# ZHKKKe/PixelSSL

Hardware: NVIDIA H100
Metric: images/sec DeepLab-v2-R101 MT 513x513 bs16 (higher is better)
Workload: dtype f16x3 (fp16 pairs, fp32 accumulate)

## Files before the change

include/pixelssl_b200.h:

```cpp
#ifndef PIXELSSL_B200_H
#define PIXELSSL_B200_H

#include <stdint.h>

#ifdef __cplusplus
extern "C" {
#endif

#define PXL_ERR_BAD_ARG   (-1)
#define PXL_ERR_UNSUPPORTED (-2)

int pxl_abi_version(void);
int64_t pxl_launch_count(void);
void pxl_reset_launch_count(void);

int64_t pxl_mse_workspace_bytes(void);
int pxl_mse_consistency(const float* s, const float* t, int64_t n, float loss_scale,
                        float* loss_out, float* grad_s, void* workspace, void* stream);
int pxl_mse_consistency_bwd(const float* s, const float* t, int64_t n, float loss_scale,
                            const float* upstream, float* grad_s, void* stream);

int pxl_ce2d(const float* logits, const float* labels, int n, int C, int64_t HW, int ignore_index,
             float* per_sample, float* grad_logits, const float* upstream, float upstream_const,
             void* stream);
// ... 60 lines not shown
int pxl_bn_bwd_params(const double* dsums, int C, float* dgamma, float* dbeta, int accumulate,
                      void* stream);

int pxl_maxpool3x3s2_fwd(const float* x, float* y, int N, int H, int W, int C, int OH, int OW,
                         void* stream);
int pxl_maxpool3x3s2_bwd(const float* x, const float* y, const float* dy, float* dx,
                         int N, int H, int W, int C, int OH, int OW, void* stream);

typedef struct {
    int N, H, W, Cin;
    int OH, OW, Cout;
    int ldo;
    int mul, div;
    int ntaps;
    int precision;
} pxl_conv_geom;
#define PXL_MAX_TAPS 64
int pxl_conv_nhwc(const pxl_conv_geom* geom_host, const int* taps_dydx_host ,
                  const float* in, const float* w, const float* bias ,
                  float* out, void* stream);
int pxl_conv_wgrad_nhwc(const pxl_conv_geom* geom_host, const int* taps_dydx_host,
                        const float* in, const float* dy, float* dw, void* stream);
int pxl_conv_tc_launch(const pxl_conv_geom* geom_host, const int* taps_dydx_host, const float* in_hi,
                       const float* in_lo, const float* w_hi, const float* w_lo, const float* bias,
                       float* out, void* stream);
typedef struct {
    int w_ntaps;
    const int* widx_host;
    int out_mul, out_offy, out_offx, out_H, out_W;
    double* bn_stats;
    float out_scale;
    const float* out_scale_dev;
    int out_accumulate;
} pxl_conv_tc_ext;
int pxl_conv_tc_launch_ex(const pxl_conv_geom* geom_host, const int* taps_dydx_host, const pxl_conv_tc_ext* ext_host,
                          const float* in_hi, const float* in_lo, const float* w_hi, const float* w_lo,
                          const float* bias, float* out, void* stream);
int pxl_conv_wgrad_tc_launch(const pxl_conv_geom* geom_host, const int* taps_dydx_host, const float* in_hi,
                             const float* in_lo, const float* dy_hi, const float* dy_lo, float* dw,
                             void* stream);
int pxl_conv_h16_launch(const pxl_conv_geom* geom_host, const int* taps_dydx_host, const pxl_conv_tc_ext* ext_host,
                        const void* in_hi, const void* in_lo, const void* w_hi, const void* w_lo,
                        const float* bias, float* out, void* stream);
int pxl_conv_wgrad_h16_launch(const pxl_conv_geom* geom_host, const int* taps_dydx_host, const void* in_hi,
                              const void* in_lo, const void* dy_hi, const void* dy_lo, float* dw, float out_scale,
                              const float* out_scale_dev, void* stream);
int pxl_h16_split(const float* x, void* hi, void* lo, int64_t n, float scale, float* slot, int target_log2,
                  void* stream);
int pxl_h16_absmax(const float* x, int64_t n, float* slot, void* stream);
int* pxl_h16_sat_counter(void);
int pxl_h16_status(void);
int pxl_h16_status_sites(int* out4_host);
int pxl_h16_reset_status(void);
int pxl_split_tf32(const float* x, float* hi, float* lo, int64_t n, void* stream);
int pxl_conv_tc_status(void);
int pxl_conv_transpose_weights(const float* w, float* wt, int Cout, int T, int Cin, void* stream);
int pxl_conv_transpose_weights_batched(const float* src_base, float* dst_base, const int64_t* table, int n,
                                       int64_t total_tiles, void* stream);
int pxl_bias_grad(const float* dy, int64_t rows, int Cout, int ldo, float* dbias, int accumulate,
                  void* stream);

int pxl_stem_conv7x7s2(const float* img_planar, const float* w, float* out, int N, int H, int W,
                       int OH, int OW, void* stream);
int pxl_stem_conv7x7s2_wgrad(const float* img_planar, const float* dy, float* dw, int N, int H, int W,
                             int OH, int OW, void* stream);
int pxl_stem_im2col(const float* img_planar, float* cols, int N, int H, int W, int OH, int OW, void* stream);

// ... 88 lines not shown
```

pixelssl_b200/_lib.py:

```python
import ctypes
import os

_HERE = os.path.dirname(os.path.abspath(__file__))
LIB_PATH = os.path.join(_HERE, 'lib', 'libpixelssl_b200.so')

c_void_p, c_int, c_int64, c_float, c_double = (ctypes.c_void_p, ctypes.c_int, ctypes.c_int64,
                                               ctypes.c_float, ctypes.c_double)


class ConvGeom(ctypes.Structure):
    _fields_ = [('N', c_int), ('H', c_int), ('W', c_int), ('Cin', c_int),
                ('OH', c_int), ('OW', c_int), ('Cout', c_int), ('ldo', c_int),
                ('mul', c_int), ('div', c_int), ('ntaps', c_int), ('precision', c_int)]


class ConvTcExt(ctypes.Structure):
    _fields_ = [('w_ntaps', c_int), ('widx_host', ctypes.POINTER(c_int)), ('out_mul', c_int),
                ('out_offy', c_int), ('out_offx', c_int), ('out_H', c_int), ('out_W', c_int),
                ('bn_stats', c_void_p), ('out_scale', c_float), ('out_scale_dev', c_void_p), ('out_accumulate', c_int)]


P = c_void_p
SIGNATURES = {
    'pxl_abi_version': (c_int, []),
    'pxl_launch_count': (c_int64, []),
    'pxl_reset_launch_count': (None, []),
    'pxl_mse_workspace_bytes': (c_int64, []),
    'pxl_mse_consistency': (c_int, [P, P, c_int64, c_float, P, P, P, P]),
    'pxl_mse_consistency_bwd': (c_int, [P, P, c_int64, c_float, P, P, P]),
    'pxl_ce2d': (c_int, [P, P, c_int, c_int, c_int64, c_int, P, P, P, c_float, P]),
    'pxl_cps_ce': (c_int, [P, P, P, P, c_int, c_int, c_int64, c_float, P, P, P, P]),
    'pxl_unimatch_ce': (c_int, [P, P, P, P, P, c_int, c_int, c_int, c_int, c_int, c_int, c_float, c_float, c_float, c_float,
                                P, P, P, P]),
    'pxl_softmax_planar': (c_int, [P, P, c_int, c_int, c_int64, P]),
    'pxl_softmax_planar_bwd': (c_int, [P, P, P, c_int, c_int, c_int64, P]),
    'pxl_softmax_mse': (c_int, [P, P, c_int, c_int, c_int64, c_float, P, P, P, P, P]),
    'pxl_bilinear_fwd': (c_int, [P, P, c_int, c_int, c_int, c_int, c_int, c_int, c_int, c_int, c_int, P]),
    'pxl_bilinear_bwd': (c_int, [P, P, c_int, c_int, c_int, c_int, c_int, c_int, c_int, c_int, c_int, P]),
    'pxl_cutmix_mix': (c_int, [P, P, P, P, c_int, c_int, c_int64, P]),
    'pxl_cutmix_confidence': (c_int, [P, c_int, c_int, c_int64, c_float, P, P]),
    'pxl_bn_stats': (c_int, [P, c_int64, c_int, P, P]),
    'pxl_bn_finalize': (c_int, [P, c_double, c_int, P, P, P, P, c_float, c_float, c_int, P, P, P, P, P]),
    'pxl_bn_eval_coeffs': (c_int, [c_int, P, P, P, P, c_float, P, P, P]),
    'pxl_bn_apply': (c_int, [P, P, P, P, c_int, P, c_int64, c_int, P]),
    'pxl_bn_bwd_reduce': (c_int, [P, P, P, P, P, c_int, c_int64, c_int, P, P, P, P]),
    'pxl_bn_bwd_dx': (c_int, [P, P, P, P, P, P, P, c_double, c_int, P, P, c_int64, c_int, P, P, P, P, P]),
    'pxl_bn_finalize_apply': (c_int, [P, P, c_double, P, P, P, P, c_float, c_float, c_int, P, P, P, P, P, c_int, P, c_int64,
                                      c_int, P]),
    'pxl_bn_bwd_params': (c_int, [P, c_int, P, P, c_int, P]),
    'pxl_bn_apply_h16': (c_int, [P, P, P, P, c_int, P, c_int64, c_int, P, P, c_float, P, P]),
    'pxl_bn_finalize_apply_h16': (c_int, [P, P, c_double, P, P, P, P, c_float, c_float, c_int, P, P, P, P, P, c_int, P, c_int64,
                                          c_int, P, P, c_float, P, P]),
    'pxl_bn_bwd_reduce_h16': (c_int, [P, P, P, P, P, c_int, c_int64, c_int, P, P, P, P, P, P]),
    'pxl_bn_bwd_dx_h16': (c_int, [P, P, P, P, P, P, P, c_double, c_int, P, P, c_int64, c_int, P, P, P, P, P, P, P, c_int, P, P]),
    'pxl_maxpool3x3s2_fwd': (c_int, [P, P, c_int, c_int, c_int, c_int, c_int, c_int, P]),
    'pxl_maxpool3x3s2_bwd': (c_int, [P, P, P, P, c_int, c_int, c_int, c_int, c_int, c_int, P]),
    'pxl_conv_nhwc': (c_int, [ctypes.POINTER(ConvGeom), ctypes.POINTER(c_int), P, P, P, P, P]),
    'pxl_conv_wgrad_nhwc': (c_int, [ctypes.POINTER(ConvGeom), ctypes.POINTER(c_int), P, P, P, P]),
    'pxl_conv_tc_launch': (c_int, [ctypes.POINTER(ConvGeom), ctypes.POINTER(c_int), P, P, P, P, P, P, P]),
    'pxl_conv_tc_launch_ex': (c_int, [ctypes.POINTER(ConvGeom), ctypes.POINTER(c_int), ctypes.POINTER(ConvTcExt), P, P, P, P, P, P, P]),
    'pxl_conv_wgrad_tc_launch': (c_int, [ctypes.POINTER(ConvGeom), ctypes.POINTER(c_int), P, P, P, P, P, P]),
    'pxl_conv_h16_launch': (c_int, [ctypes.POINTER(ConvGeom), ctypes.POINTER(c_int), ctypes.POINTER(ConvTcExt), P, P, P, P, P, P, P]),
    'pxl_conv_wgrad_h16_launch': (c_int, [ctypes.POINTER(ConvGeom), ctypes.POINTER(c_int), P, P, P, P, P, c_float, P, P]),
    'pxl_h16_split': (c_int, [P, P, P, c_int64, c_float, P, c_int, P]),
    'pxl_h16_absmax': (c_int, [P, c_int64, P, P]),
    'pxl_h16_sat_counter': (c_void_p, []),
    'pxl_h16_status': (c_int, []),
    'pxl_h16_status_sites': (c_int, [P]),
    'pxl_h16_reset_status': (c_int, []),
    'pxl_split_tf32': (c_int, [P, P, P, c_int64, P]),
    'pxl_conv_tc_status': (c_int, []),
    'pxl_conv_transpose_weights': (c_int, [P, P, c_int, c_int, c_int, P]),
    'pxl_conv_transpose_weights_batched': (c_int, [P, P, P, c_int, c_int64, P]),
    'pxl_bias_grad': (c_int, [P, c_int64, c_int, c_int, P, c_int, P]),
    'pxl_stem_conv7x7s2': (c_int, [P, P, P, c_int, c_int, c_int, c_int, c_int, P]),
    'pxl_stem_conv7x7s2_wgrad': (c_int, [P, P, P, c_int, c_int, c_int, c_int, c_int, P]),
    'pxl_stem_im2col': (c_int, [P, P, c_int, c_int, c_int, c_int, c_int, P]),
    'pxl_planar_to_nhwc': (c_int, [P, P, c_int, c_int, c_int64, c_int, c_int, P]),
    'pxl_nhwc_to_planar': (c_int, [P, P, c_int, c_int, c_int64, c_int, c_int, P]),
    'pxl_onehot_nhwc': (c_int, [P, P, c_int64, c_int, c_int, c_int, P]),
    'pxl_leaky_relu_fwd': (c_int, [P, P, c_int64, c_float, P]),
    'pxl_leaky_relu_bwd': (c_int, [P, P, P, c_int64, c_float, P]),
    'pxl_bce_logits_masked': (c_int, [P, P, c_float, c_int, c_int, c_int64, P, P, P, c_float, P]),
    'pxl_adam': (c_int, [P, P, P, P, c_int64, c_float, c_float, c_float, c_float, c_float, c_int, P]),
    'pxl_gauss_blur_sep': (c_int, [P, P, P, c_int, c_int, c_int, c_int, P, c_float, P]),
    'pxl_dilate3x3_reflect': (c_int, [P, P, c_int, c_int, c_int, P]),
    'pxl_minmax_norm': (c_int, [P, P, c_int, c_int64, c_float, c_float, c_float, P]),
    'pxl_gct_dcgt': (c_int, [P, P, P, P, c_float, c_int, c_int, c_int64, P, P, P, P]),
    'pxl_fdgt_absdiff': (c_int, [P, P, c_float, c_int, c_int, c_int64, P, P]),
    'pxl_pixel_shuffle2_nhwc': (c_int, [P, P, c_int, c_int, c_int, c_int, c_int, c_int, c_int, P]),
    'pxl_perturb_nhwc': (c_int, [P, P, P, P, P, c_int, c_int64, c_int, P]),
    'pxl_fp_dup_nhwc': (c_int, [P, P, P, c_int, c_int64, c_int, P]),
    'pxl_fp_dup_bwd_nhwc': (c_int, [P, P, P, c_int, c_int64, c_int, P]),
    'pxl_channel_mean_nhwc': (c_int, [P, P, c_int64, c_int, P]),
# ... 74 lines not shown
```

pixelssl_b200/csrc/common.cuh:

```cuda
#pragma once
#include <cuda_runtime.h>
#include <stdint.h>
#include "../../include/pixelssl_b200.h"

#define PXL_NUM_SMS 132

extern "C" void pxl_count_launch_(int n);

#define PXL_WS_WGRAD 0
#define PXL_WS_BIAS 1
#define PXL_WS_CE 2
#define PXL_WS_CPS 3
#define PXL_WS_UNIMATCH 4
#define PXL_WS_STRONG_AUG 5
#define PXL_WS_PURPOSES 6
#define PXL_WS_STREAMS 8
extern "C" void* pxl_workspace_(int purpose, void* stream, size_t bytes, int* rc);

#define PXL_CHECK_LAUNCH()                                   \
    do {                                                     \
        pxl_count_launch_(1);                                \
        cudaError_t e__ = cudaPeekAtLastError();             \
        if (e__ != cudaSuccess) return (int)e__;             \
    } while (0)

static inline int64_t pxl_cdiv(int64_t a, int64_t b) { return (a + b - 1) / b; }

#define PXL_PDL_SYNC()                                                   \
    do {                                                                 \
        asm volatile("griddepcontrol.launch_dependents;" ::: "memory");  \
        asm volatile("griddepcontrol.wait;" ::: "memory");               \
    } while (0)

extern "C" int pxl_pdl_enabled_(void);

template <typename... KArgs, typename... Args>
static inline cudaError_t pxl_launch_pdl(void (*kernel)(KArgs...), dim3 grid, dim3 block, size_t smem, cudaStream_t st,
                                         Args&&... args) {
    cudaLaunchConfig_t cfg = {};
    cfg.gridDim = grid; cfg.blockDim = block; cfg.dynamicSmemBytes = smem; cfg.stream = st;
    cudaLaunchAttribute at[1];
    at[0].id = cudaLaunchAttributeProgrammaticStreamSerialization;
    at[0].val.programmaticStreamSerializationAllowed = 1;
    cfg.attrs = at; cfg.numAttrs = pxl_pdl_enabled_() ? 1 : 0;
    return cudaLaunchKernelEx(&cfg, kernel, static_cast<KArgs>(args)...);
}

__device__ __forceinline__ float warp_sum(float v) {
// ... 36 lines not shown
```

pixelssl_b200/csrc/conv_tc.cu:

```cuda
#include "common.cuh"
#include <cuda.h>
#include <cstdlib>
#include <type_traits>

typedef CUresult (*EncodeTiledFn)(CUtensorMap*, CUtensorMapDataType, cuuint32_t, void*, const cuuint64_t*,
                                  const cuuint64_t*, const cuuint32_t*, const cuuint32_t*, CUtensorMapInterleave,
                                  CUtensorMapSwizzle, CUtensorMapL2promotion, CUtensorMapFloatOOBfill);
static EncodeTiledFn get_encode() {
    static EncodeTiledFn fn = nullptr;
    if (!fn) {
        void* p = nullptr;
        cudaDriverEntryPointQueryResult q;
        if (cudaGetDriverEntryPoint("cuTensorMapEncodeTiled", &p, cudaEnableDefault, &q) == cudaSuccess &&
            q == cudaDriverEntryPointSuccess)
            fn = (EncodeTiledFn)p;
    }
    return fn;
}

static int make_act_map(CUtensorMap* m, const void* base, int C, int W, int H, int N, int bw, int bh, int estride = 1, int f16 = 0) {
    EncodeTiledFn enc = get_encode();
    if (!enc) return PXL_ERR_UNSUPPORTED;
    const cuuint64_t eb = f16 ? 2 : 4;
    cuuint64_t dims[4] = {(cuuint64_t)C, (cuuint64_t)W, (cuuint64_t)H, (cuuint64_t)N};
// ... 158 lines not shown
#pragma unroll
    for (int k = 0; k < 4; ++k) wgmma_op<BN, F16>(part, da + 2 * k, db + 2 * k, k);
    if (split3) {
#pragma unroll
        for (int k = 0; k < 4; ++k) wgmma_op<BN, F16>(corr, dal + 2 * k, db + 2 * k, k);
#pragma unroll
        for (int k = 0; k < 4; ++k) wgmma_op<BN, F16>(corr, da + 2 * k, dbl + 2 * k, 1);
    }
}

__device__ __forceinline__ float4 tf32_split4(float4 v, float4& lo) {
    float4 h;
    const float* vp = &v.x; float* hp = &h.x; float* lp = &lo.x;
#pragma unroll
    for (int e = 0; e < 4; ++e) {
        uint32_t u;
        asm("cvt.rna.tf32.f32 %0, %1;" : "=r"(u) : "f"(vp[e]));
        u &= 0xFFFFE000u;
        hp[e] = __uint_as_float(u);
        lp[e] = vp[e] - hp[e];
    }
    return h;
}

struct TcParams {
    int Cin, Cout, ldo, ntaps, kchunks;
    int N, OH, OW;
    int BW, BH, tilesW, tilesH;
    int stages, nsplit;
    int a_inkernel;
    int in_mul;
    int out_mul, out_offy, out_offx, outH, outW;
    int ntilesN, pix_tiles, total_tiles;
    int kc;
    float out_scale;
    int out_acc;
    short dy[PXL_MAX_TAPS], dx[PXL_MAX_TAPS], widx[PXL_MAX_TAPS];
};

#define TC_A_BYTES (128 * 128)
#define TC_MAX_STAGES 8
#define TC_THREADS 384

__device__ __forceinline__ void tc_tile_coords(const TcParams& p, int tile, int bn, int& n0, int& w0, int& h0, int& n) {
    const int nt = tile / p.pix_tiles, pix = tile - nt * p.pix_tiles;
    const int tw = pix % p.tilesW, th = (pix / p.tilesW) % p.tilesH;
    n = pix / (p.tilesW * p.tilesH);
    w0 = tw * p.BW; h0 = th * p.BH; n0 = nt * bn;
}

template <int BN, int F16>
__global__ void __launch_bounds__(TC_THREADS, 1)
conv_wg_kernel(const __grid_constant__ CUtensorMap mapA, const __grid_constant__ CUtensorMap mapAlo,
               const __grid_constant__ CUtensorMap mapB, const __grid_constant__ CUtensorMap mapBlo,
               const TcParams p, const float* __restrict__ bias, float* __restrict__ out,
               double* __restrict__ stats, int* __restrict__ err_flag, const float* __restrict__ oscale_ptr) {
    extern __shared__ __align__(1024) uint8_t smem_raw[];
    __shared__ uint64_t full_bar[TC_MAX_STAGES], empty_bar[TC_MAX_STAGES];
    __shared__ float st_warp[2][8][BN];

    uint8_t* smem = (uint8_t*)(((uintptr_t)smem_raw + 1023) & ~(uintptr_t)1023);
    constexpr int B_BYTES = BN * 128;
    constexpr int PER_OP = TC_A_BYTES + B_BYTES;
    const int stage_bytes = PER_OP * (p.nsplit == 3 ? 2 : 1);
    const int iters = p.ntaps * p.kchunks;

    if (threadIdx.x == 0) {
        for (int s = 0; s < p.stages; ++s) { mbar_init(&full_bar[s], 1); mbar_init(&empty_bar[s], 256); }
        asm volatile("fence.mbarrier_init.release.cluster;" ::: "memory");
    }
    __syncthreads();
    PXL_PDL_SYNC();

    if (threadIdx.x < 128) {
        asm volatile("setmaxnreg.dec.sync.aligned.u32 40;" ::: "memory");
        if (threadIdx.x >= 32) return;
        uint32_t tx = (uint32_t)((p.BW * p.BH * 128 + B_BYTES) * (p.nsplit == 3 ? 2 : 1));
        if (p.a_inkernel) tx -= (uint32_t)(p.BW * p.BH * 128);
        uint32_t s = 0, ph = 0;
        bool ok = true;
        for (int tile = blockIdx.x; tile < p.total_tiles && ok; tile += gridDim.x) {
            int n0, w0, h0, n;
            tc_tile_coords(p, tile, BN, n0, w0, h0, n);
            int tap = 0, c0 = 0;
            for (int it = 0; it < iters; ++it) {
                ok = __all_sync(0xffffffffu, mbar_wait(&empty_bar[s], ph ^ 1u, err_flag, 1));
                if (!ok) break;
                uint8_t* sa = smem + (size_t)s * stage_bytes;
                const int ax = w0 * p.in_mul + p.dx[tap], ay = h0 * p.in_mul + p.dy[tap];
// ... 73 lines not shown
            } else {
                asm volatile("wgmma.wait_group.sync.aligned 1;" ::: "memory");
                fence_regs(corr);
                if (it > 0) {
                    mbar_arrive(&empty_bar[prev]);
#pragma unroll
                    for (int i = 0; i < BN / 2; ++i) acc[i] += corr[i];
                }
                wg_arrive();
                fence_regs(corr);
#pragma unroll
                for (int k = 2; k < 4; ++k) wgmma_op<BN, 1>(corr, da + 2 * k, db + 2 * k, k - 2);
                wg_commit();
                asm volatile("wgmma.wait_group.sync.aligned 1;" ::: "memory");
                fence_regs(part);
#pragma unroll
                for (int i = 0; i < BN / 2; ++i) acc[i] += part[i];
            }
            prev = s;
            if (++s == (uint32_t)p.stages) { s = 0; ph ^= 1u; }
        }
        if (!S3) {
            wg_wait0();
            fence_regs(corr);
            mbar_arrive(&empty_bar[prev]);
#pragma unroll
            for (int i = 0; i < BN / 2; ++i) acc[i] += corr[i];
        }
        return true;
    };
    for (int tile = blockIdx.x; tile < p.total_tiles && ok; tile += gridDim.x) {
        int n0, w0, h0, n;
        tc_tile_coords(p, tile, BN, n0, w0, h0, n);
        if (stats && n0 != st_n0) { flush_stats(); st_n0 = n0; }
#pragma unroll
        for (int i = 0; i < BN / 2; ++i) acc[i] = 0.f;
        if constexpr (F16 != 0) ok = split3 ? f16_tile(std::true_type{}) : f16_tile(std::false_type{});
        else for (int it = 0; it < iters; ++it) {
            ok = __all_sync(0xffffffffu, mbar_wait(&full_bar[s], ph, err_flag, 2));
            if (!ok) break;
            uint8_t* sa = smem + (size_t)s * stage_bytes;
            if (p.a_inkernel) {
                float4* a_hi = reinterpret_cast<float4*>(sa + cw * (TC_A_BYTES / 2));
                float4* a_lo = reinterpret_cast<float4*>(sa + PER_OP + cw * (TC_A_BYTES / 2));
#pragma unroll
                for (int c = 0; c < TC_A_BYTES / 2 / 16 / 128; ++c) {
                    float4 lo;
                    const float4 hi = tf32_split4(a_hi[t + c * 128], lo);
                    a_hi[t + c * 128] = hi;
                    a_lo[t + c * 128] = lo;
                }
                fence_async_smem();
                named_bar(2 + cw, 128);
            }
            const uint32_t sa32 = smem_base + s * (uint32_t)stage_bytes;
            const uint32_t arow = (uint32_t)cw * (TC_A_BYTES / 2);
            const uint64_t da = sw128_desc(sa32 + arow), db = sw128_desc(sa32 + TC_A_BYTES);
            const uint64_t dal = sw128_desc(sa32 + PER_OP + arow), dbl = sw128_desc(sa32 + PER_OP + TC_A_BYTES);
            wg_arrive();
            fence_regs(part);
            fence_regs(corr);
#pragma unroll
            for (int k = 0; k < 2; ++k) wgmma_op<BN, F16>(part, da + 2 * k, db + 2 * k, k);
            if (split3) {
#pragma unroll
                for (int k = 0; k < 4; ++k) wgmma_op<BN, F16>(corr, dal + 2 * k, db + 2 * k, k);
#pragma unroll
// ... 53 lines not shown
                } else if (c1ok && vec2) {
                    *reinterpret_cast<float2*>(o) = make_float2(v[h][0], v[h][1]);
                } else {
                    if (c0ok) o[0] = v[h][0];
                    if (c1ok) o[1] = v[h][1];
                }
            }
            if (stats) {
                float s0 = (valid[0] ? v[0][0] : 0.f) + (valid[1] ? v[1][0] : 0.f);
                float s1 = (valid[0] ? v[0][1] : 0.f) + (valid[1] ? v[1][1] : 0.f);
                float q0 = (valid[0] ? v[0][0] * v[0][0] : 0.f) + (valid[1] ? v[1][0] * v[1][0] : 0.f);
                float q1 = (valid[0] ? v[0][1] * v[0][1] : 0.f) + (valid[1] ? v[1][1] * v[1][1] : 0.f);
#pragma unroll
                for (int o = 4; o < 32; o <<= 1) {
                    s0 += __shfl_xor_sync(0xffffffffu, s0, o); s1 += __shfl_xor_sync(0xffffffffu, s1, o);
                    q0 += __shfl_xor_sync(0xffffffffu, q0, o); q1 += __shfl_xor_sync(0xffffffffu, q1, o);
                }
                if (lane < 4) {
                    const int slot = cw * 4 + warp;
                    st_warp[0][slot][cl] = s0; st_warp[0][slot][cl + 1] = s1;
                    st_warp[1][slot][cl] = q0; st_warp[1][slot][cl + 1] = q1;
                }
            }
        }
        if (stats) {
            named_bar(1, 256);
            if (ct < BN) {
#pragma unroll
                for (int w8 = 0; w8 < 8; ++w8) { st_s += st_warp[0][w8][ct]; st_q += st_warp[1][w8][ct]; }
            }
            named_bar(1, 256);
        }
    }
    if (stats && ok) flush_stats();
}

__global__ void __launch_bounds__(256)
split_tf32_kernel(const float4* __restrict__ x, float4* __restrict__ hi, float4* __restrict__ lo, int64_t n4) {
    const int64_t stride = (int64_t)gridDim.x * blockDim.x;
    for (int64_t i = (int64_t)blockIdx.x * blockDim.x + threadIdx.x; i < n4; i += stride) {
        float4 l;
        hi[i] = tf32_split4(__ldcs(x + i), l);
        lo[i] = l;
    }
}

extern "C" int pxl_split_tf32(const float* x, float* hi, float* lo, int64_t n, void* stream) {
    if (!x || !hi || !lo || n <= 0 || (n & 3)) return PXL_ERR_BAD_ARG;
    const int64_t n4 = n / 4;
    int blocks = (int)(pxl_cdiv(n4, 256 * 2) < PXL_NUM_SMS * 8 ? pxl_cdiv(n4, 256 * 2) : PXL_NUM_SMS * 8);
    split_tf32_kernel<<<blocks, 256, 0, (cudaStream_t)stream>>>((const float4*)x, (float4*)hi, (float4*)lo, n4);
    PXL_CHECK_LAUNCH();
    return 0;
}

static int* g_err_flag = nullptr;

static int ensure_err_flag() {
    if (g_err_flag) return 0;
    cudaError_t e = cudaMalloc(&g_err_flag, sizeof(int));
    if (e != cudaSuccess) return (int)e;
    e = cudaMemset(g_err_flag, 0, sizeof(int));
    return e == cudaSuccess ? 0 : (int)e;
}

template <typename K>
static int query_dyn_smem_limit(K kernel) {
    int dev = 0, optin = 0;
    cudaFuncAttributes a;
    if (cudaGetDevice(&dev) != cudaSuccess || cudaDeviceGetAttribute(&optin, cudaDevAttrMaxSharedMemoryPerBlockOptin, dev) != cudaSuccess ||
        cudaFuncGetAttributes(&a, kernel) != cudaSuccess)
        return 0;
    return optin - (int)a.sharedSizeBytes;
}

static void pick_tile(int OH, int OW, bool flat, int& BW, int& BH) {
    if (flat) { BW = 128; BH = 1; return; }
    double best = -1.0;
    BW = 16; BH = 8;
    for (int bw = 4; bw <= 128 && bw <= 256; ++bw) {
        int bh = 128 / bw;
        if (bh < 1) break;
        if (bh > 256) bh = 256;
        const int64_t tiles = (int64_t)((OW + bw - 1) / bw) * ((OH + bh - 1) / bh);
        const double eff = (double)OH * OW / ((double)tiles * 128.0);
        if (eff > best + 1e-9) { best = eff; BW = bw; BH = bh; }
    }
}

template <int BN, int F16>
static int fwd_smem_limit() {
    static const int v = query_dyn_smem_limit(conv_wg_kernel<BN, F16>);
    return v;
}

template <int BN, int F16>
static int launch_fwd(const CUtensorMap& mA, const CUtensorMap& mAlo, const CUtensorMap& mB, const CUtensorMap& mBlo,
                      const TcParams& p, size_t smem, cudaStream_t st, const float* bias, float* out, double* stats,
                      const float* oscale_ptr) {
    static bool attr = false;
    if (!attr) {
        cudaError_t e = cudaFuncSetAttribute(conv_wg_kernel<BN, F16>, cudaFuncAttributeMaxDynamicSharedMemorySize, fwd_smem_limit<BN, F16>());
        if (e != cudaSuccess) return (int)e;
        attr = true;
    }
    const unsigned nblk = (unsigned)(p.total_tiles < PXL_NUM_SMS ? p.total_tiles : PXL_NUM_SMS);
    cudaError_t le = pxl_launch_pdl(conv_wg_kernel<BN, F16>, dim3(nblk), dim3(TC_THREADS), smem, st, mA, mAlo, mB, mBlo, p,
                                    bias, out, stats, g_err_flag, oscale_ptr);
    if (le != cudaSuccess) return (int)le;
    PXL_CHECK_LAUNCH();
    return 0;
}

static int conv_tc_launch_core(const pxl_conv_geom* g, const int* taps, const pxl_conv_tc_ext* ext,
                               const void* in_hi, const void* in_lo, const void* w_hi, const void* w_lo,
                               const float* bias, float* out, void* stream);

extern "C" int pxl_conv_tc_launch(const pxl_conv_geom* g, const int* taps, const float* in_hi, const float* in_lo,
                                  const float* w_hi, const float* w_lo, const float* bias, float* out, void* stream) {
    if (g && g->precision > 2) return PXL_ERR_BAD_ARG;
    return conv_tc_launch_core(g, taps, nullptr, in_hi, in_lo, w_hi, w_lo, bias, out, stream);
}

extern "C" int pxl_conv_tc_launch_ex(const pxl_conv_geom* g, const int* taps, const pxl_conv_tc_ext* ext,
                                     const float* in_hi, const float* in_lo, const float* w_hi, const float* w_lo,
                                     const float* bias, float* out, void* stream) {
    if (g && g->precision > 2) return PXL_ERR_BAD_ARG;
    return conv_tc_launch_core(g, taps, ext, in_hi, in_lo, w_hi, w_lo, bias, out, stream);
}

extern "C" int pxl_conv_h16_launch(const pxl_conv_geom* g, const int* taps, const pxl_conv_tc_ext* ext,
                                   const void* in_hi, const void* in_lo, const void* w_hi, const void* w_lo,
                                   const float* bias, float* out, void* stream) {
    if (!g || (g->precision != 3 && g->precision != 4)) return PXL_ERR_BAD_ARG;
    return conv_tc_launch_core(g, taps, ext, in_hi, in_lo, w_hi, w_lo, bias, out, stream);
}

static int conv_tc_launch_core(const pxl_conv_geom* g, const int* taps, const pxl_conv_tc_ext* ext,
                               const void* in_hi, const void* in_lo, const void* w_hi, const void* w_lo,
                               const float* bias, float* out, void* stream) {
    if (!g || !taps || !in_hi || !w_hi || !out) return PXL_ERR_BAD_ARG;
    if ((g->mul != 1 && g->mul != 2) || g->div != 1) return PXL_ERR_UNSUPPORTED;
    const int f16 = g->precision >= 3 ? 1 : 0;
    const int kc = f16 ? 64 : 32;
    if (g->Cin % kc != 0 || g->ntaps > PXL_MAX_TAPS) return PXL_ERR_UNSUPPORTED;
    const int wtaps = ext && ext->w_ntaps > 0 ? ext->w_ntaps : g->ntaps;
    const int nsplit = (g->precision == 2 || g->precision == 3) ? 3 : 1;
    if (nsplit == 3 && !w_lo) return PXL_ERR_BAD_ARG;
    if (f16 && nsplit == 3 && !in_lo) return PXL_ERR_BAD_ARG;
    const int a_inkernel = (!f16 && nsplit == 3 && !in_lo) ? 1 : 0;
    const int omul = (ext && ext->out_mul > 0) ? ext->out_mul : 1;
    const bool has_out_xform = ext && (omul != 1 || ext->out_offy != 0 || ext->out_offx != 0);
    bool flat = (g->ntaps == 1 && taps[0] == 0 && taps[1] == 0 && g->OH == g->H && g->OW == g->W && g->mul == 1 &&
                 !has_out_xform);
    TcParams p;
    p.Cin = g->Cin; p.Cout = g->Cout; p.ldo = g->ldo; p.ntaps = g->ntaps; p.kchunks = g->Cin / kc;
    p.nsplit = nsplit; p.a_inkernel = a_inkernel; p.kc = kc;
    p.out_scale = (ext && ext->out_scale != 0.f) ? ext->out_scale : 1.f;
    const float* oscale_ptr = ext ? ext->out_scale_dev : nullptr;
    for (int t = 0; t < g->ntaps; ++t) {
        p.dy[t] = (short)taps[2 * t]; p.dx[t] = (short)taps[2 * t + 1];
        p.widx[t] = (short)((ext && ext->widx_host) ? ext->widx_host[t] : t);
        if (p.widx[t] < 0 || p.widx[t] >= wtaps) return PXL_ERR_BAD_ARG;
    }
    p.in_mul = g->mul;
    p.out_mul = omul; p.out_offy = has_out_xform ? ext->out_offy : 0; p.out_offx = has_out_xform ? ext->out_offx : 0;
    int mapW, mapH, mapN;
    if (flat) {
        const int64_t M = (int64_t)g->N * g->H * g->W;
        if (M >= (1ll << 31)) return PXL_ERR_UNSUPPORTED;
        p.N = 1; p.OH = 1; p.OW = (int)M;
        mapW = (int)M; mapH = 1; mapN = 1;
        p.outH = 1; p.outW = (int)M;
    } else {
        p.N = g->N; p.OH = g->OH; p.OW = g->OW;
        mapW = g->W; mapH = g->H; mapN = g->N;
        p.outH = has_out_xform ? ext->out_H : g->OH; p.outW = has_out_xform ? ext->out_W : g->OW;
    }
    pick_tile(p.OH, p.OW, flat, p.BW, p.BH);
    if (g->mul == 2 && (p.BW > 128 || p.BH > 128)) return PXL_ERR_UNSUPPORTED;
    const int BN = g->Cout > 64 ? 128 : (g->Cout > 32 ? 64 : 32);
    const int stage_bytes = (TC_A_BYTES + BN * 128) * (nsplit == 3 ? 2 : 1);
    p.tilesW = (p.OW + p.BW - 1) / p.BW; p.tilesH = (p.OH + p.BH - 1) / p.BH;
    p.pix_tiles = p.N * p.tilesH * p.tilesW;
    p.ntilesN = (g->Cout + BN - 1) / BN;
    const int64_t n_tiles = (int64_t)p.pix_tiles * p.ntilesN;
    if (n_tiles >= (1ll << 31)) return PXL_ERR_UNSUPPORTED;
    p.total_tiles = (int)n_tiles;
    const int smem_limit = f16 ? (BN == 128 ? fwd_smem_limit<128, 1>() : BN == 64 ? fwd_smem_limit<64, 1>() : fwd_smem_limit<32, 1>())
                               : (BN == 128 ? fwd_smem_limit<128, 0>() : BN == 64 ? fwd_smem_limit<64, 0>() : fwd_smem_limit<32, 0>());
    if (smem_limit <= 0) return PXL_ERR_UNSUPPORTED;
    p.stages = (smem_limit - 1024) / stage_bytes;
    if (p.stages > TC_MAX_STAGES) p.stages = TC_MAX_STAGES;
    if (p.stages < 2) return PXL_ERR_UNSUPPORTED;
    const size_t smem = (size_t)p.stages * stage_bytes + 1024;

    CUtensorMap mA, mAlo, mB, mBlo;
    int rc = make_act_map(&mA, in_hi, g->Cin, mapW, mapH, mapN, p.BW, p.BH, g->mul, f16);
    if (rc) return rc;
    rc = make_w_map(&mB, w_hi, (int64_t)wtaps * g->Cin, g->Cout, BN, f16);
    if (rc) return rc;
    if (nsplit == 3) {
        if (a_inkernel) mAlo = mA;
        else {
            rc = make_act_map(&mAlo, in_lo, g->Cin, mapW, mapH, mapN, p.BW, p.BH, g->mul, f16);
            if (rc) return rc;
        }
        rc = make_w_map(&mBlo, w_lo, (int64_t)wtaps * g->Cin, g->Cout, BN, f16);
        if (rc) return rc;
    } else {
        mAlo = mA; mBlo = mB;
    }
    p.out_acc = (ext && ext->out_accumulate) ? 1 : 0;
    if ((rc = ensure_err_flag())) return rc;
    cudaStream_t st = (cudaStream_t)stream;
    double* st_ptr = ext ? (double*)ext->bn_stats : nullptr;
    if (f16) {
        if (BN == 128) return launch_fwd<128, 1>(mA, mAlo, mB, mBlo, p, smem, st, bias, out, st_ptr, oscale_ptr);
        if (BN == 64) return launch_fwd<64, 1>(mA, mAlo, mB, mBlo, p, smem, st, bias, out, st_ptr, oscale_ptr);
        return launch_fwd<32, 1>(mA, mAlo, mB, mBlo, p, smem, st, bias, out, st_ptr, oscale_ptr);
    }
    if (BN == 128) return launch_fwd<128, 0>(mA, mAlo, mB, mBlo, p, smem, st, bias, out, st_ptr, oscale_ptr);
    if (BN == 64) return launch_fwd<64, 0>(mA, mAlo, mB, mBlo, p, smem, st, bias, out, st_ptr, oscale_ptr);
    return launch_fwd<32, 0>(mA, mAlo, mB, mBlo, p, smem, st, bias, out, st_ptr, oscale_ptr);
}

extern "C" int pxl_conv_tc_status(void) {
    if (!g_err_flag) return 0;
    int v = 0;
    if (cudaMemcpy(&v, g_err_flag, sizeof(int), cudaMemcpyDeviceToHost) != cudaSuccess) return -1;
    return v;
}

extern "C" int pxl_conv_tc_impl(const pxl_conv_geom* g, const int* taps, const float* in, const float* w,
                                const float* bias, float* out, void* stream) {
    if (!g) return PXL_ERR_BAD_ARG;
    if (g->precision == 2) return PXL_ERR_UNSUPPORTED;
    return pxl_conv_tc_launch(g, taps, in, nullptr, w, nullptr, bias, out, stream);
}

struct WgParams {
    int Cin, Cout, ldo, ntaps;
    int N, OH, OW, mul;
    int BW, BH, tilesW, tilesH, rows, rows_alloc;
    int stages, nsplit;
    int inkernel;
    int slab_ch;
    float out_scale;
    int tiles_ci, ktiles_per_cta, ktiles_total;
    short dy[PXL_MAX_TAPS], dx[PXL_MAX_TAPS];
};

template <int BN, int F16>
__global__ void __launch_bounds__(TC_THREADS, 1)
conv_wgrad_wg_kernel(const __grid_constant__ CUtensorMap mapDy, const __grid_constant__ CUtensorMap mapDyLo,
                     const __grid_constant__ CUtensorMap mapX, const __grid_constant__ CUtensorMap mapXLo,
                     const WgParams p, float* __restrict__ dw, float* __restrict__ ws, int* __restrict__ err_flag,
// ... 386 lines not shown
```

pixelssl_b200/ops.py:

```python
import ctypes
import functools

import torch

from . import _lib
from ._lib import ConvGeom, ConvTcExt, call
from .nn.peer import MAX_VALUES as _PEER_MAX_VALUES

CL = torch.channels_last
PRECISION = {'fp32': 0, 'tf32': 1, 'tf32x3': 2, 'f16x3': 3, 'f16': 4}
H16_FALLBACK = {3: 2, 4: 1}
H16_ACT_SCALE = 16.0
H16_W_SCALE = 256.0
H16_GRAD_TARGET_LOG2 = 14
_conv_precision = 0


def set_conv_precision(name):
    global _conv_precision
    _conv_precision = PRECISION[name]


def get_conv_precision():
    return _conv_precision
# ... 561 lines not shown
    return transpose_weights(w, *shape) if transposed else w


@functools.lru_cache(maxsize=None)
def conv_route(direction, Cin, Cout, mul, div, precision):
    if direction == 'wgrad':
        strides_ok, chans = div == 1 and mul in (1, 2), (Cin, Cout)
    else:
        strides_ok, chans = (div == 1 and mul in (1, 2)) or (div == 2 and mul == 1), (Cin,)
    if precision >= 3:
        if strides_ok and all(c % 64 == 0 for c in chans):
            return 'h16', precision
        precision = H16_FALLBACK[precision]
    if precision != 0 and strides_ok and all(c % 32 == 0 for c in chans):
        return 'tc', precision
    return 'ffma', 0


def _stride2_dgrad_classes(taps, ntaps):
    classes = []
    for py in (0, 1):
        for px in (0, 1):
            sub, widx = [], []
            for t in range(ntaps):
                dy, dx = taps[2 * t], taps[2 * t + 1]
                if (py + dy) % 2 == 0 and (px + dx) % 2 == 0:
                    sub += [(py + dy) // 2, (px + dx) // 2]
                    widx.append(t)
            classes.append((py, px, sub, widx))
    return classes


def conv_raw(x, w_packed, bias, taps, N, H, W, Cin, OH, OW, Cout, ldo, mul, div, out=None, precision=None, bn_stats=None,
             accumulate=False):
    ntaps = len(taps) // 2
    family, prec = conv_route('fwd', Cin, Cout, mul, div, _conv_precision if precision is None else precision)
    if family != 'h16' and (isinstance(x, H16) or isinstance(w_packed, H16)):
        raise ValueError('fp16-pair operands given for a shape the f16 wgmma kernel does not cover')
    if out is None:
        out = torch.empty((N, ldo, OH, OW), dtype=torch.float32, device=(x[0] if isinstance(x, tuple) else x).device,
                          memory_format=CL)
        if ldo != Cout:
            out.zero_()
    if family == 'ffma':
        if isinstance(x, tuple):
            x = x[0] + x[1]
        if isinstance(w_packed, tuple):
            w_packed = w_packed[0] + w_packed[1]
        geom = ConvGeom(N, H, W, Cin, OH, OW, Cout, ldo, mul, div, ntaps, 0)
        call('pxl_conv_nhwc', ctypes.byref(geom), _ctaps(taps), _p(x), _p(w_packed), _p(bias), _p(out), _stream())
        return out
    if div == 1:
        ext = None
        if bn_stats is not None or family == 'h16':
            ext = ConvTcExt(0, None, 0, 0, 0, 0, 0, _p(bn_stats))
        if bn_stats is not None:
            bn_stats._pxl_filled = True
        launches = [(ConvGeom(N, H, W, Cin, OH, OW, Cout, ldo, mul, 1, ntaps, prec), taps, ext)]
    else:
        launches = []
        classes = _stride2_dgrad_classes(taps, ntaps)
        if any(len(c[3]) == 0 for c in classes):
            out.zero_()
        for py, px, sub, widx in classes:
            ohs, ows = (OH - py + 1) // 2, (OW - px + 1) // 2
            if widx and ohs > 0 and ows > 0:
                launches.append((ConvGeom(N, H, W, Cin, ohs, ows, Cout, ldo, 1, 1, len(widx), prec), sub,
                                 ConvTcExt(ntaps, (ctypes.c_int * len(widx))(*widx), 2, py, px, OH, OW, None)))
    if family == 'h16':
        want_lo = prec == 3
        xh = x if isinstance(x, H16) else _pair_of(x, want_lo)
        wh = w_packed if isinstance(w_packed, H16) else conv_weight(w_packed, 'h16', (Cout, ntaps, Cin), want_lo=want_lo)
        fx, px = xh.inv_scale()
        fw, pw = wh.inv_scale()
        if px is not None and pw is not None:
            raise ValueError('at most one operand may carry a device-side scale')
        oscale, odev = fx * fw, _p(px if px is not None else pw)
        for geom, tp, ext in launches:
            ext.out_scale, ext.out_scale_dev, ext.out_accumulate = oscale, odev, 1 if accumulate else 0
            _timed_call('pxl_conv_h16_launch', ctypes.byref(geom), _ctaps(tp), ctypes.byref(ext), _p(xh.hi), _p(xh.lo),
                        _p(wh.hi), _p(wh.lo if want_lo else None), _p(bias), _p(out), _stream(),
                        meta=(2.0 * geom.N * geom.OH * geom.OW * geom.Cin * geom.Cout * geom.ntaps,
                              'fwd/dgrad N%d %dx%d Cin%d Cout%d taps%d mul%d' % (geom.N, geom.OH, geom.OW, geom.Cin, geom.Cout, geom.ntaps, geom.mul)))
        return out
    x_parts = x if isinstance(x, tuple) else (x, None)
    if prec == 2:
        w_parts = w_packed if isinstance(w_packed, tuple) else conv_weight(w_packed, 'split', (Cout, ntaps, Cin))
    else:
        w_parts = (w_packed, None)
    for geom, tp, ext in launches:
        _timed_call('pxl_conv_tc_launch_ex', ctypes.byref(geom), _ctaps(tp), ctypes.byref(ext) if ext is not None else None,
                    _p(x_parts[0]), _p(x_parts[1]), _p(w_parts[0]), _p(w_parts[1]), _p(bias), _p(out), _stream(),
                    meta=(2.0 * geom.N * geom.OH * geom.OW * geom.Cin * geom.Cout * geom.ntaps,
                          'fwd/dgrad(tf32) N%d %dx%d Cin%d Cout%d taps%d' % (geom.N, geom.OH, geom.OW, geom.Cin, geom.Cout, geom.ntaps)))
    return out


def conv_tc_status():
    return int(_lib.load().pxl_conv_tc_status())


# ... 1167 lines not shown
```

Baseline: 167.2.

## Split conv wave-quantization tail into narrower-N launch with BN-stats handoff

Adds a tail schedule for the tensor-core conv: when the tile count does not divide evenly across SMs, the full waves run with 128-wide N tiles and the remainder runs as a second launch using 64- or 32-wide N tiles, so more SMs share the tail. A cost model picks wide, tail64 or tail32 automatically for f16 paths with large K. BN statistics from the last head tiles are carried to the tail launch through a workspace buffer so their partial sums are not flushed twice. This costs an extra launch, extra tensor-map setup, and more complex stats bookkeeping. Narrower tiles also reuse the A operand less.

```diff
diff --git a/include/pixelssl_b200.h b/include/pixelssl_b200.h
--- a/include/pixelssl_b200.h
+++ b/include/pixelssl_b200.h
@@ -116,7 +116,13 @@
     float out_scale;
     const float* out_scale_dev;
     int out_accumulate;
+    int schedule;
 } pxl_conv_tc_ext;
+#define PXL_CONV_SCHED_AUTO 0
+#define PXL_CONV_SCHED_WIDE 1
+#define PXL_CONV_SCHED_TAIL64 2
+#define PXL_CONV_SCHED_TAIL32 3
+int pxl_conv_tc_schedule(const pxl_conv_geom* geom_host, const int* taps_dydx_host, const pxl_conv_tc_ext* ext_host);
 int pxl_conv_tc_launch_ex(const pxl_conv_geom* geom_host, const int* taps_dydx_host, const pxl_conv_tc_ext* ext_host,
                           const float* in_hi, const float* in_lo, const float* w_hi, const float* w_lo,
                           const float* bias, float* out, void* stream);
diff --git a/pixelssl_b200/_lib.py b/pixelssl_b200/_lib.py
--- a/pixelssl_b200/_lib.py
+++ b/pixelssl_b200/_lib.py
@@ -17,7 +17,8 @@
 class ConvTcExt(ctypes.Structure):
     _fields_ = [('w_ntaps', c_int), ('widx_host', ctypes.POINTER(c_int)), ('out_mul', c_int),
                 ('out_offy', c_int), ('out_offx', c_int), ('out_H', c_int), ('out_W', c_int),
-                ('bn_stats', c_void_p), ('out_scale', c_float), ('out_scale_dev', c_void_p), ('out_accumulate', c_int)]
+                ('bn_stats', c_void_p), ('out_scale', c_float), ('out_scale_dev', c_void_p), ('out_accumulate', c_int),
+                ('schedule', c_int)]
 
 
 P = c_void_p
@@ -60,6 +61,7 @@
     'pxl_conv_tc_launch': (c_int, [ctypes.POINTER(ConvGeom), ctypes.POINTER(c_int), P, P, P, P, P, P, P]),
     'pxl_conv_tc_launch_ex': (c_int, [ctypes.POINTER(ConvGeom), ctypes.POINTER(c_int), ctypes.POINTER(ConvTcExt), P, P, P, P, P, P, P]),
     'pxl_conv_wgrad_tc_launch': (c_int, [ctypes.POINTER(ConvGeom), ctypes.POINTER(c_int), P, P, P, P, P, P]),
+    'pxl_conv_tc_schedule': (c_int, [ctypes.POINTER(ConvGeom), ctypes.POINTER(c_int), ctypes.POINTER(ConvTcExt)]),
     'pxl_conv_h16_launch': (c_int, [ctypes.POINTER(ConvGeom), ctypes.POINTER(c_int), ctypes.POINTER(ConvTcExt), P, P, P, P, P, P, P]),
     'pxl_conv_wgrad_h16_launch': (c_int, [ctypes.POINTER(ConvGeom), ctypes.POINTER(c_int), P, P, P, P, P, c_float, P, P]),
     'pxl_h16_split': (c_int, [P, P, P, c_int64, c_float, P, c_int, P]),
diff --git a/pixelssl_b200/csrc/common.cuh b/pixelssl_b200/csrc/common.cuh
--- a/pixelssl_b200/csrc/common.cuh
+++ b/pixelssl_b200/csrc/common.cuh
@@ -13,7 +13,8 @@
 #define PXL_WS_CPS 3
 #define PXL_WS_UNIMATCH 4
 #define PXL_WS_STRONG_AUG 5
-#define PXL_WS_PURPOSES 6
+#define PXL_WS_CONV_TAIL 6
+#define PXL_WS_PURPOSES 7
 #define PXL_WS_STREAMS 8
 extern "C" void* pxl_workspace_(int purpose, void* stream, size_t bytes, int* rc);
 
diff --git a/pixelssl_b200/csrc/conv_tc.cu b/pixelssl_b200/csrc/conv_tc.cu
--- a/pixelssl_b200/csrc/conv_tc.cu
+++ b/pixelssl_b200/csrc/conv_tc.cu
@@ -214,6 +214,9 @@
     int in_mul;
     int out_mul, out_offy, out_offx, outH, outW;
     int ntilesN, pix_tiles, total_tiles;
+    int tile_base, sub;
+    int ho_out;
+    int ho_in;
     int kc;
     float out_scale;
     int out_acc;
@@ -225,10 +228,11 @@
 #define TC_THREADS 384
 
 __device__ __forceinline__ void tc_tile_coords(const TcParams& p, int tile, int bn, int& n0, int& w0, int& h0, int& n) {
-    const int nt = tile / p.pix_tiles, pix = tile - nt * p.pix_tiles;
+    const int q = tile / p.sub, t = p.tile_base + q;
+    const int nt = t / p.pix_tiles, pix = t - nt * p.pix_tiles;
     const int tw = pix % p.tilesW, th = (pix / p.tilesW) % p.tilesH;
     n = pix / (p.tilesW * p.tilesH);
-    w0 = tw * p.BW; h0 = th * p.BH; n0 = nt * bn;
+    w0 = tw * p.BW; h0 = th * p.BH; n0 = (nt * p.sub + tile - q * p.sub) * bn;
 }
 
 template <int BN, int F16>
@@ -236,7 +240,8 @@
 conv_wg_kernel(const __grid_constant__ CUtensorMap mapA, const __grid_constant__ CUtensorMap mapAlo,
                const __grid_constant__ CUtensorMap mapB, const __grid_constant__ CUtensorMap mapBlo,
                const TcParams p, const float* __restrict__ bias, float* __restrict__ out,
-               double* __restrict__ stats, int* __restrict__ err_flag, const float* __restrict__ oscale_ptr) {
+               double* __restrict__ stats, int* __restrict__ err_flag, const float* __restrict__ oscale_ptr,
+               float* __restrict__ handoff) {
     extern __shared__ __align__(1024) uint8_t smem_raw[];
     __shared__ uint64_t full_bar[TC_MAX_STAGES], empty_bar[TC_MAX_STAGES];
     __shared__ float st_warp[2][8][BN];
@@ -376,7 +381,11 @@
     for (int tile = blockIdx.x; tile < p.total_tiles && ok; tile += gridDim.x) {
         int n0, w0, h0, n;
         tc_tile_coords(p, tile, BN, n0, w0, h0, n);
-        if (stats && n0 != st_n0) { flush_stats(); st_n0 = n0; }
+        if (stats && p.ho_in) {
+            flush_stats(); st_n0 = n0;
+            const int q = tile / p.sub, c = (tile - q * p.sub) * BN + ct;
+            if (handoff && ct < BN) { st_s = __ldcg(handoff + q * 256 + c); st_q = __ldcg(handoff + q * 256 + 128 + c); }
+        } else if (stats && n0 != st_n0) { flush_stats(); st_n0 = n0; }
 #pragma unroll
         for (int i = 0; i < BN / 2; ++i) acc[i] = 0.f;
         if constexpr (F16 != 0) ok = split3 ? f16_tile(std::true_type{}) : f16_tile(std::false_type{});
@@ -496,7 +505,14 @@
             named_bar(1, 256);
         }
     }
-    if (stats && ok) flush_stats();
+    if (stats && ok) {
+        if ((int)blockIdx.x < p.ho_out) {
+            if ((p.total_tiles + (int)blockIdx.x) / p.pix_tiles * BN != st_n0) flush_stats();
+            if (ct < BN) { handoff[blockIdx.x * 256 + ct] = st_s; handoff[blockIdx.x * 256 + 128 + ct] = st_q; }
+        } else {
+            flush_stats();
+        }
+    }
 }
 
 __global__ void __launch_bounds__(256)
@@ -561,7 +577,7 @@
 template <int BN, int F16>
 static int launch_fwd(const CUtensorMap& mA, const CUtensorMap& mAlo, const CUtensorMap& mB, const CUtensorMap& mBlo,
                       const TcParams& p, size_t smem, cudaStream_t st, const float* bias, float* out, double* stats,
-                      const float* oscale_ptr) {
+                      const float* oscale_ptr, float* handoff) {
     static bool attr = false;
     if (!attr) {
         cudaError_t e = cudaFuncSetAttribute(conv_wg_kernel<BN, F16>, cudaFuncAttributeMaxDynamicSharedMemorySize, fwd_smem_limit<BN, F16>());
@@ -570,7 +586,7 @@
     }
     const unsigned nblk = (unsigned)(p.total_tiles < PXL_NUM_SMS ? p.total_tiles : PXL_NUM_SMS);
     cudaError_t le = pxl_launch_pdl(conv_wg_kernel<BN, F16>, dim3(nblk), dim3(TC_THREADS), smem, st, mA, mAlo, mB, mBlo, p,
-                                    bias, out, stats, g_err_flag, oscale_ptr);
+                                    bias, out, stats, g_err_flag, oscale_ptr, handoff);
     if (le != cudaSuccess) return (int)le;
     PXL_CHECK_LAUNCH();
     return 0;
@@ -600,28 +616,24 @@
     return conv_tc_launch_core(g, taps, ext, in_hi, in_lo, w_hi, w_lo, bias, out, stream);
 }
 
-static int conv_tc_launch_core(const pxl_conv_geom* g, const int* taps, const pxl_conv_tc_ext* ext,
-                               const void* in_hi, const void* in_lo, const void* w_hi, const void* w_lo,
-                               const float* bias, float* out, void* stream) {
-    if (!g || !taps || !in_hi || !w_hi || !out) return PXL_ERR_BAD_ARG;
+static int tc_width(int Cout) { return Cout > 64 ? 128 : (Cout > 32 ? 64 : 32); }
+
+static int tc_plan(const pxl_conv_geom* g, const int* taps, const pxl_conv_tc_ext* ext, TcParams& p, int& mapW, int& mapH,
+                   int& mapN) {
+    if (!g || !taps) return PXL_ERR_BAD_ARG;
+    if (ext && (ext->schedule < PXL_CONV_SCHED_AUTO || ext->schedule > PXL_CONV_SCHED_TAIL32)) return PXL_ERR_BAD_ARG;
     if ((g->mul != 1 && g->mul != 2) || g->div != 1) return PXL_ERR_UNSUPPORTED;
     const int f16 = g->precision >= 3 ? 1 : 0;
     const int kc = f16 ? 64 : 32;
     if (g->Cin % kc != 0 || g->ntaps > PXL_MAX_TAPS) return PXL_ERR_UNSUPPORTED;
     const int wtaps = ext && ext->w_ntaps > 0 ? ext->w_ntaps : g->ntaps;
-    const int nsplit = (g->precision == 2 || g->precision == 3) ? 3 : 1;
-    if (nsplit == 3 && !w_lo) return PXL_ERR_BAD_ARG;
-    if (f16 && nsplit == 3 && !in_lo) return PXL_ERR_BAD_ARG;
-    const int a_inkernel = (!f16 && nsplit == 3 && !in_lo) ? 1 : 0;
     const int omul = (ext && ext->out_mul > 0) ? ext->out_mul : 1;
     const bool has_out_xform = ext && (omul != 1 || ext->out_offy != 0 || ext->out_offx != 0);
     bool flat = (g->ntaps == 1 && taps[0] == 0 && taps[1] == 0 && g->OH == g->H && g->OW == g->W && g->mul == 1 &&
                  !has_out_xform);
-    TcParams p;
     p.Cin = g->Cin; p.Cout = g->Cout; p.ldo = g->ldo; p.ntaps = g->ntaps; p.kchunks = g->Cin / kc;
-    p.nsplit = nsplit; p.a_inkernel = a_inkernel; p.kc = kc;
+    p.nsplit = (g->precision == 2 || g->precision == 3) ? 3 : 1; p.a_inkernel = 0; p.kc = kc;
     p.out_scale = (ext && ext->out_scale != 0.f) ? ext->out_scale : 1.f;
-    const float* oscale_ptr = ext ? ext->out_scale_dev : nullptr;
     for (int t = 0; t < g->ntaps; ++t) {
         p.dy[t] = (short)taps[2 * t]; p.dx[t] = (short)taps[2 * t + 1];
         p.widx[t] = (short)((ext && ext->widx_host) ? ext->widx_host[t] : t);
@@ -629,7 +641,6 @@
     }
     p.in_mul = g->mul;
     p.out_mul = omul; p.out_offy = has_out_xform ? ext->out_offy : 0; p.out_offx = has_out_xform ? ext->out_offx : 0;
-    int mapW, mapH, mapN;
     if (flat) {
         const int64_t M = (int64_t)g->N * g->H * g->W;
         if (M >= (1ll << 31)) return PXL_ERR_UNSUPPORTED;
@@ -643,50 +654,112 @@
     }
     pick_tile(p.OH, p.OW, flat, p.BW, p.BH);
     if (g->mul == 2 && (p.BW > 128 || p.BH > 128)) return PXL_ERR_UNSUPPORTED;
-    const int BN = g->Cout > 64 ? 128 : (g->Cout > 32 ? 64 : 32);
-    const int stage_bytes = (TC_A_BYTES + BN * 128) * (nsplit == 3 ? 2 : 1);
     p.tilesW = (p.OW + p.BW - 1) / p.BW; p.tilesH = (p.OH + p.BH - 1) / p.BH;
     p.pix_tiles = p.N * p.tilesH * p.tilesW;
-    p.ntilesN = (g->Cout + BN - 1) / BN;
-    const int64_t n_tiles = (int64_t)p.pix_tiles * p.ntilesN;
+    p.ntilesN = (g->Cout + tc_width(g->Cout) - 1) / tc_width(g->Cout);
+    const int64_t n_tiles = (int64_t)p.pix_tiles * p.ntilesN * (128 / 32);
     if (n_tiles >= (1ll << 31)) return PXL_ERR_UNSUPPORTED;
-    p.total_tiles = (int)n_tiles;
-    const int smem_limit = f16 ? (BN == 128 ? fwd_smem_limit<128, 1>() : BN == 64 ? fwd_smem_limit<64, 1>() : fwd_smem_limit<32, 1>())
-                               : (BN == 128 ? fwd_smem_limit<128, 0>() : BN == 64 ? fwd_smem_limit<64, 0>() : fwd_smem_limit<32, 0>());
-    if (smem_limit <= 0) return PXL_ERR_UNSUPPORTED;
-    p.stages = (smem_limit - 1024) / stage_bytes;
-    if (p.stages > TC_MAX_STAGES) p.stages = TC_MAX_STAGES;
-    if (p.stages < 2) return PXL_ERR_UNSUPPORTED;
-    const size_t smem = (size_t)p.stages * stage_bytes + 1024;
-
-    CUtensorMap mA, mAlo, mB, mBlo;
-    int rc = make_act_map(&mA, in_hi, g->Cin, mapW, mapH, mapN, p.BW, p.BH, g->mul, f16);
+    p.total_tiles = p.pix_tiles * p.ntilesN;
+    p.tile_base = 0; p.sub = 1; p.ho_out = 0; p.ho_in = 0;
+    return 0;
+}
+
+static const double kTcWave64 = 0.55, kTcWave32 = 0.28, kTcTailLaunch = 0.25;
+static const int kTcMinK = 512;
+
+static int tc_auto_schedule(int64_t T, int K, int f16) {
+    if (!f16 || K < kTcMinK) return PXL_CONV_SCHED_WIDE;
+    const int64_t S = PXL_NUM_SMS, full = T / S, r = T % S;
+    if (r == 0) return PXL_CONV_SCHED_WIDE;
+    const double head = full ? full + kTcTailLaunch : 0.0;
+    const double c64 = head + pxl_cdiv(2 * r, S) * kTcWave64, c32 = head + pxl_cdiv(4 * r, S) * kTcWave32;
+    if (c32 < c64 && c32 < full + 1) return PXL_CONV_SCHED_TAIL32;
+    return c64 < full + 1 ? PXL_CONV_SCHED_TAIL64 : PXL_CONV_SCHED_WIDE;
+}
+
+static int tc_schedule(const pxl_conv_geom* g, const TcParams& p, const pxl_conv_tc_ext* ext) {
+    if (tc_width(g->Cout) != 128) return PXL_CONV_SCHED_WIDE;
+    const int forced = ext ? ext->schedule : 0;
+    return forced != PXL_CONV_SCHED_AUTO ? forced : tc_auto_schedule(p.total_tiles, g->Cin * g->ntaps, g->precision >= 3);
+}
+
+extern "C" int pxl_conv_tc_schedule(const pxl_conv_geom* g, const int* taps, const pxl_conv_tc_ext* ext) {
+    TcParams p;
+    int mapW, mapH, mapN;
+    const int rc = tc_plan(g, taps, ext, p, mapW, mapH, mapN);
+    return rc ? rc : tc_schedule(g, p, ext);
+}
+
+static int conv_tc_launch_core(const pxl_conv_geom* g, const int* taps, const pxl_conv_tc_ext* ext,
+                               const void* in_hi, const void* in_lo, const void* w_hi, const void* w_lo,
+                               const float* bias, float* out, void* stream) {
+    if (!g || !taps || !in_hi || !w_hi || !out) return PXL_ERR_BAD_ARG;
+    TcParams p;
+    int mapW, mapH, mapN;
+    int rc = tc_plan(g, taps, ext, p, mapW, mapH, mapN);
     if (rc) return rc;
-    rc = make_w_map(&mB, w_hi, (int64_t)wtaps * g->Cin, g->Cout, BN, f16);
+    const int f16 = g->precision >= 3 ? 1 : 0;
+    const int wtaps = ext && ext->w_ntaps > 0 ? ext->w_ntaps : g->ntaps;
+    const int nsplit = p.nsplit;
+    if (nsplit == 3 && !w_lo) return PXL_ERR_BAD_ARG;
+    if (f16 && nsplit == 3 && !in_lo) return PXL_ERR_BAD_ARG;
+    p.a_inkernel = (!f16 && nsplit == 3 && !in_lo) ? 1 : 0;
+    p.out_acc = (ext && ext->out_accumulate) ? 1 : 0;
+    const float* oscale_ptr = ext ? ext->out_scale_dev : nullptr;
+
+    CUtensorMap mA, mAlo;
+    rc = make_act_map(&mA, in_hi, g->Cin, mapW, mapH, mapN, p.BW, p.BH, g->mul, f16);
     if (rc) return rc;
-    if (nsplit == 3) {
-        if (a_inkernel) mAlo = mA;
-        else {
-            rc = make_act_map(&mAlo, in_lo, g->Cin, mapW, mapH, mapN, p.BW, p.BH, g->mul, f16);
-            if (rc) return rc;
-        }
-        rc = make_w_map(&mBlo, w_lo, (int64_t)wtaps * g->Cin, g->Cout, BN, f16);
+    if (nsplit == 3 && !p.a_inkernel) {
+        rc = make_act_map(&mAlo, in_lo, g->Cin, mapW, mapH, mapN, p.BW, p.BH, g->mul, f16);
         if (rc) return rc;
     } else {
-        mAlo = mA; mBlo = mB;
-    }
-    p.out_acc = (ext && ext->out_accumulate) ? 1 : 0;
+        mAlo = mA;
+    }
     if ((rc = ensure_err_flag())) return rc;
     cudaStream_t st = (cudaStream_t)stream;
     double* st_ptr = ext ? (double*)ext->bn_stats : nullptr;
-    if (f16) {
-        if (BN == 128) return launch_fwd<128, 1>(mA, mAlo, mB, mBlo, p, smem, st, bias, out, st_ptr, oscale_ptr);
-        if (BN == 64) return launch_fwd<64, 1>(mA, mAlo, mB, mBlo, p, smem, st, bias, out, st_ptr, oscale_ptr);
-        return launch_fwd<32, 1>(mA, mAlo, mB, mBlo, p, smem, st, bias, out, st_ptr, oscale_ptr);
-    }
-    if (BN == 128) return launch_fwd<128, 0>(mA, mAlo, mB, mBlo, p, smem, st, bias, out, st_ptr, oscale_ptr);
-    if (BN == 64) return launch_fwd<64, 0>(mA, mAlo, mB, mBlo, p, smem, st, bias, out, st_ptr, oscale_ptr);
-    return launch_fwd<32, 0>(mA, mAlo, mB, mBlo, p, smem, st, bias, out, st_ptr, oscale_ptr);
+    const int T = p.total_tiles;
+    auto run = [&](int bn, int t0, int t1, int ho_out, int ho_in, float* ho) -> int {
+        TcParams q = p;
+        q.sub = tc_width(g->Cout) / bn; q.tile_base = t0; q.total_tiles = (t1 - t0) * q.sub;
+        q.ho_out = ho_out; q.ho_in = ho_in;
+        const int stage_bytes = (TC_A_BYTES + bn * 128) * (nsplit == 3 ? 2 : 1);
+        const int smem_limit = f16 ? (bn == 128 ? fwd_smem_limit<128, 1>() : bn == 64 ? fwd_smem_limit<64, 1>() : fwd_smem_limit<32, 1>())
+                                   : (bn == 128 ? fwd_smem_limit<128, 0>() : bn == 64 ? fwd_smem_limit<64, 0>() : fwd_smem_limit<32, 0>());
+        if (smem_limit <= 0) return PXL_ERR_UNSUPPORTED;
+        q.stages = (smem_limit - 1024) / stage_bytes;
+        if (q.stages > TC_MAX_STAGES) q.stages = TC_MAX_STAGES;
+        if (q.stages < 2) return PXL_ERR_UNSUPPORTED;
+        const size_t smem = (size_t)q.stages * stage_bytes + 1024;
+        CUtensorMap mB, mBlo;
+        int e = make_w_map(&mB, w_hi, (int64_t)wtaps * g->Cin, g->Cout, bn, f16);
+        if (e) return e;
+        if (nsplit == 3) {
+            if ((e = make_w_map(&mBlo, w_lo, (int64_t)wtaps * g->Cin, g->Cout, bn, f16))) return e;
+        } else {
+            mBlo = mB;
+        }
+        if (f16) {
+            if (bn == 128) return launch_fwd<128, 1>(mA, mAlo, mB, mBlo, q, smem, st, bias, out, st_ptr, oscale_ptr, ho);
+            if (bn == 64) return launch_fwd<64, 1>(mA, mAlo, mB, mBlo, q, smem, st, bias, out, st_ptr, oscale_ptr, ho);
+            return launch_fwd<32, 1>(mA, mAlo, mB, mBlo, q, smem, st, bias, out, st_ptr, oscale_ptr, ho);
+        }
+        if (bn == 128) return launch_fwd<128, 0>(mA, mAlo, mB, mBlo, q, smem, st, bias, out, st_ptr, oscale_ptr, ho);
+        if (bn == 64) return launch_fwd<64, 0>(mA, mAlo, mB, mBlo, q, smem, st, bias, out, st_ptr, oscale_ptr, ho);
+        return launch_fwd<32, 0>(mA, mAlo, mB, mBlo, q, smem, st, bias, out, st_ptr, oscale_ptr, ho);
+    };
+    const int sched = tc_schedule(g, p, ext);
+    if (sched == PXL_CONV_SCHED_WIDE) return run(tc_width(g->Cout), 0, T, 0, 0, nullptr);
+    const int head = T / PXL_NUM_SMS * PXL_NUM_SMS, r = T - head;
+    if (r == 0) return run(128, 0, T, 0, 0, nullptr);
+    float* ho = nullptr;
+    if (head > 0 && st_ptr) {
+        ho = (float*)pxl_workspace_(PXL_WS_CONV_TAIL, stream, (size_t)PXL_NUM_SMS * 256 * sizeof(float), &rc);
+        if (rc) return rc;
+    }
+    if (head > 0 && (rc = run(128, 0, head, ho ? r : 0, 0, ho))) return rc;
+    return run(sched == PXL_CONV_SCHED_TAIL64 ? 64 : 32, head, T, 0, 1, ho);
 }
 
 extern "C" int pxl_conv_tc_status(void) {
diff --git a/pixelssl_b200/ops.py b/pixelssl_b200/ops.py
--- a/pixelssl_b200/ops.py
+++ b/pixelssl_b200/ops.py
@@ -617,7 +617,7 @@
 
 
 def conv_raw(x, w_packed, bias, taps, N, H, W, Cin, OH, OW, Cout, ldo, mul, div, out=None, precision=None, bn_stats=None,
-             accumulate=False):
+             accumulate=False, schedule=0):
     ntaps = len(taps) // 2
     family, prec = conv_route('fwd', Cin, Cout, mul, div, _conv_precision if precision is None else precision)
     if family != 'h16' and (isinstance(x, H16) or isinstance(w_packed, H16)):
@@ -637,7 +637,7 @@
         return out
     if div == 1:
         ext = None
-        if bn_stats is not None or family == 'h16':
+        if bn_stats is not None or family == 'h16' or schedule:
             ext = ConvTcExt(0, None, 0, 0, 0, 0, 0, _p(bn_stats))
         if bn_stats is not None:
             bn_stats._pxl_filled = True
@@ -652,6 +652,9 @@
             if widx and ohs > 0 and ows > 0:
                 launches.append((ConvGeom(N, H, W, Cin, ohs, ows, Cout, ldo, 1, 1, len(widx), prec), sub,
                                  ConvTcExt(ntaps, (ctypes.c_int * len(widx))(*widx), 2, py, px, OH, OW, None)))
+    for _, _, ext in launches:
+        if ext is not None:
+            ext.schedule = schedule
     if family == 'h16':
         want_lo = prec == 3
         xh = x if isinstance(x, H16) else _pair_of(x, want_lo)
```

After: 171.3, median of 6. 2.4% higher.
